# BrByte/brb_framework

Hardware: AMD Instinct MI355X
Metric: GiB/s (device-resident) + Mrecords/s over 1500B buffers at 1/2/4/8 MI355X (higher is better)
Workload: dtype u32

## Files before the change

brb_framework_amd/csrc/gpu/digest_var_line.h:

```cpp
#pragma once

#include "byte_stream.h"
#include "digest_line.h"
#include "test_options.h"

namespace brb_digest {

template <class Alg>
BRB_DEV typename Alg::State digest_lane(const uint8_t *a, uint64_t len)
{
    typename Alg::State st = Alg::iv();
    brb_io::BlockSrc src;
    src.init(a, len);
    uint32_t w[16];
    for (uint64_t b = 0; b < (len >> 6); ++b) {
        src.fetch(w);
        Alg::compress(st, w);
    }
    src.fetch(w);
    brb_io::add_marker(w, len);
    Alg::finish(st, w, uint32_t(len & 63), len);
    return st;
}

BRB_DEV uint64_t uniform64(uint64_t v)
{
    return (uint64_t(uint32_t(__builtin_amdgcn_readfirstlane(int(uint32_t(v >> 32))))) << 32) |
           uint32_t(__builtin_amdgcn_readfirstlane(int(uint32_t(v))));
}

BRB_DEV uint64_t wave_min64(uint64_t v)
{
#pragma unroll
    for (int m = 32; m >= 1; m >>= 1) {
        const uint64_t o = __shfl_xor(v, m, 64);
        v = o < v ? o : v;
    }
    return v;
}

BRB_DEV uint64_t wave_max64(uint64_t v)
{
#pragma unroll
    for (int m = 32; m >= 1; m >>= 1) {
        const uint64_t o = __shfl_xor(v, m, 64);
        v = o > v ? o : v;
    }
    return v;
}

constexpr uint32_t kSortCG = 4;
constexpr uint32_t kSortNB = 8;

BRB_DEV uint64_t sorted_record(uint64_t g, uint32_t lane, const uint32_t *__restrict__ lens, uint64_t n_rec,
                               uint32_t *scratch)
{
    const uint64_t cg = (g / kSortCG) * kSortCG;
    const uint64_t c0 = cg * 64;
    const uint64_t left = (n_rec + 63) / 64 - cg;
    const uint32_t pc = left < kSortCG ? uint32_t(left) : kSortCG;
    const uint32_t j = uint32_t((g % kSortCG + g / gridDim.x) % pc);
    uint32_t it[kSortCG];
    bool ok[kSortCG];
    uint32_t lo = 0xFFFFFFFFu, hi = 0;
#pragma unroll
    for (uint32_t v = 0; v < kSortCG; v++) {
        const uint64_t idx = c0 + 64 * v + lane;
        ok[v] = idx < n_rec;
        const uint32_t len = ok[v] ? lens[idx] : 0u;
        const uint32_t nb = (len >> 6) + ((len & 63) ? 1u : 0u);
        it[v] = (nb >> 1) + (nb & 1);
        lo = ok[v] && it[v] < lo ? it[v] : lo;
        hi = ok[v] && it[v] > hi ? it[v] : hi;
    }
#pragma unroll
    for (int m = 32; m >= 1; m >>= 1) {
        const uint32_t a = uint32_t(__shfl_xor(int(lo), m, 64)), b = uint32_t(__shfl_xor(int(hi), m, 64));
        lo = a < lo ? a : lo;
        hi = b > hi ? b : hi;
    }
    lo = __builtin_amdgcn_readfirstlane(lo);
    hi = __builtin_amdgcn_readfirstlane(hi);
    const uint32_t span = hi > lo ? hi - lo : 0u;
    const float scale = span < kSortNB ? 1.0f : float(kSortNB - 1) / float(span);
    uint32_t key[kSortCG], pos[kSortCG];
#pragma unroll
    for (uint32_t v = 0; v < kSortCG; v++) {
        const uint32_t d = it[v] - lo;
        const uint32_t q = uint32_t(float(d) * scale + 0.5f);
        key[v] = !ok[v] ? kSortNB - 1 : (q < kSortNB ? q : kSortNB - 1);
        pos[v] = 0;
    }
    uint32_t base = 0;
#pragma unroll
    for (uint32_t k = 0; k < kSortNB; k++) {
#pragma unroll
        for (uint32_t v = 0; v < kSortCG; v++) {
            const uint64_t m = __builtin_amdgcn_ballot_w64(key[v] == k);
            const uint32_t below = __builtin_amdgcn_mbcnt_hi(uint32_t(m >> 32), __builtin_amdgcn_mbcnt_lo(uint32_t(m), 0u));
            pos[v] = key[v] == k ? base + below : pos[v];
            base += uint32_t(__builtin_popcountll(m));
        }
    }
#pragma unroll
    for (uint32_t v = 0; v < kSortCG; v++)
        scratch[pos[v]] = ok[v] ? 64 * v + lane : 0xFFFFFFFFu;
    __builtin_amdgcn_s_waitcnt(0xC07F);
    __builtin_amdgcn_wave_barrier();
    const uint32_t e = scratch[64 * j + lane];
    __builtin_amdgcn_s_waitcnt(0xC07F);
    __builtin_amdgcn_wave_barrier();
    return e == 0xFFFFFFFFu ? ~uint64_t(0) : c0 + e;
}

template <class Alg, int WAVES, bool OUT_ALIGNED, bool FIXED = false, bool SORT = false>
__global__ __launch_bounds__(64 * WAVES, 2) void digest_var_line_kernel(const uint8_t *__restrict__ data,
                                                                        const uint64_t *__restrict__ offs,
                                                                        const uint32_t *__restrict__ lens,
                                                                        uint32_t rec_len, uint64_t n_rec,
                                                                        uint8_t *__restrict__ out,
                                                                        uint64_t brb_first_sorted = 0)
{
    constexpr uint32_t SLOT = 8192;
    constexpr uint32_t OOB = 0x80000000u;
    __shared__ __attribute__((aligned(16))) uint8_t ring[WAVES * 2 * SLOT];
    __shared__ uint32_t sort_scratch[SORT ? WAVES * 64 * kSortCG : 1];
    __shared__ uint32_t next_ticket;
    const uint32_t lane = threadIdx.x & 63;
    const uint32_t wv = __builtin_amdgcn_readfirstlane(threadIdx.x >> 6);
    const uint64_t n_groups = (n_rec + 63) / 64;
    if (threadIdx.x == 0)
        next_ticket = WAVES;
    __syncthreads();
    auto take = [&]() -> uint64_t {
        uint32_t tk = 0;
        if (lane == 0)
            tk = __hip_atomic_fetch_add(&next_ticket, 1u, __ATOMIC_RELAXED, __HIP_MEMORY_SCOPE_WORKGROUP);
        tk = __builtin_amdgcn_readfirstlane(tk);
        return uint64_t(blockIdx.x) + uint64_t(tk) * gridDim.x;
    };
    uint64_t g = uint64_t(blockIdx.x) + uint64_t(wv) * gridDim.x;
    if (g >= n_groups)
        return;
    const uint32_t my_off = wv * 2 * SLOT;
    const uint32_t lds0 = uint32_t(reinterpret_cast<uintptr_t>(ring)) + my_off;
    const uint64_t dbase = reinterpret_cast<uint64_t>(data);
    auto swz = [](uint32_t row) { return (row >> 1) & 7; };

    struct Grp {
        uint64_t a;
        uint64_t r;
        uint32_t len;
        uint32_t K;
        bool line;
        brb_dma::v4i rs;
        uint32_t vq[8];
        uint32_t lq[8];
    };
    const uint64_t first_sorted = brb_first_sorted;
    auto record_of = [&](uint64_t g) -> uint64_t {
        if (SORT && g >= first_sorted && g < n_groups)
            return sorted_record(g, lane, lens, n_rec, sort_scratch + wv * (64 * kSortCG));
        return g * 64 + lane < n_rec ? g * 64 + lane : ~uint64_t(0);
    };
    auto setup = [&](uint64_t g, uint64_t rec, Grp &G) {
        const uint64_t r = rec != ~uint64_t(0) ? rec : uniform64(g * 64);
        G.r = rec;
        G.a = dbase + (FIXED ? r * rec_len : offs[r]);
        G.len = FIXED ? rec_len : (rec != ~uint64_t(0) ? lens[r] : 0u);
        const uint64_t line = G.a & ~uint64_t(127);
        const uint32_t lines = G.len ? uint32_t(((G.a & 127) + G.len + 127) >> 7) : 0u;
        const uint32_t nblk = (G.len >> 6) + ((G.len & 63) ? 1u : 0u);
        const uint64_t lo = uniform64(wave_min64(G.len ? line : ~uint64_t(0)));
        const uint64_t hi = uniform64(wave_max64(G.len ? line + 128 * uint64_t(lines) : 0));
        G.K = __builtin_amdgcn_readfirstlane(uint32_t(wave_max64((nblk + 1) >> 1)));
        G.line = hi > lo && hi - lo < (uint64_t(1) << 31) - (uint64_t(1) << 16);
        const uint64_t base = lo - 4096;
        const uint64_t left = hi - base;
        G.rs.x = __builtin_amdgcn_readfirstlane(int(uint32_t(base)));
        G.rs.y = __builtin_amdgcn_readfirstlane(int(uint32_t(base >> 32) & 0xFFFF));
        G.rs.z = __builtin_amdgcn_readfirstlane(int(left > 0x7FFFFFFFull ? 0x7FFFFFFFu : uint32_t(left)));
        G.rs.w = 0x00020000;
        const uint32_t rel = uint32_t(line - lo);
        const uint32_t l3 = lane >> 3;
        const uint32_t g0 = 16u * ((lane & 7) ^ (l3 >> 1));
#pragma unroll
        for (int q = 0; q < 8; q++) {
            const int src = int(8 * q + l3) * 4;
            const uint32_t rrel = uint32_t(__builtin_amdgcn_ds_bpermute(src, int(rel)));
            G.lq[q] = uint32_t(__builtin_amdgcn_ds_bpermute(src, int(lines)));
            G.vq[q] = (rrel | (q & 1 ? g0 ^ 64u : g0)) + (4096u - 1024u * (q & 3));
        }
    };
    auto issue = [&](Grp &G, uint32_t m, uint32_t slot, bool keep_l2 = false) {
        const uint32_t lm = lds0 + slot * SLOT;
        uint32_t v[8];
#pragma unroll
        for (int q = 0; q < 8; q++)
            v[q] = m < G.lq[q] ? G.vq[q] : OOB;
        uint32_t keep;
#define BRB_VLINE_DMA8(POL)                                                                     \
        asm volatile("s_mov_b32 %0, m0\n\t"                                                    \
                     "s_mov_b32 m0, %10\n\t"                                                   \
                     "s_nop 0\n\t"                                                             \
                     "buffer_load_dwordx4 %1, %9, 0 offen " POL "lds\n\t"                      \
                     "buffer_load_dwordx4 %2, %9, 0 offen offset:1024 " POL "lds\n\t"          \
                     "buffer_load_dwordx4 %3, %9, 0 offen offset:2048 " POL "lds\n\t"          \
                     "buffer_load_dwordx4 %4, %9, 0 offen offset:3072 " POL "lds\n\t"          \
                     "s_mov_b32 m0, %11\n\t"                                                   \
                     "s_nop 0\n\t"                                                             \
                     "buffer_load_dwordx4 %5, %9, 0 offen " POL "lds\n\t"                      \
                     "buffer_load_dwordx4 %6, %9, 0 offen offset:1024 " POL "lds\n\t"          \
                     "buffer_load_dwordx4 %7, %9, 0 offen offset:2048 " POL "lds\n\t"          \
                     "buffer_load_dwordx4 %8, %9, 0 offen offset:3072 " POL "lds\n\t"          \
                     "s_mov_b32 m0, %0"                                                         \
                     : "=&s"(keep)                                                              \
                     : "v"(v[0]), "v"(v[1]), "v"(v[2]), "v"(v[3]), "v"(v[4]), "v"(v[5]), "v"(v[6]), "v"(v[7]), \
                       "s"(G.rs), "s"(lm), "s"(lm + 4096u)                                      \
                     : "memory")
        if (keep_l2)
            BRB_VLINE_DMA8("");
        else
            BRB_VLINE_DMA8("nt ");
#undef BRB_VLINE_DMA8
        const uint64_t b = ((uint64_t(uint32_t(G.rs.y)) << 32) | uint32_t(G.rs.x)) + 128u;
        G.rs.x = int(uint32_t(b));
        G.rs.y = int(uint32_t(b >> 32));
        int z = G.rs.z;
        asm("s_sub_i32 %0, %0, 0x80\n\ts_max_i32 %0, %0, 0" : "+s"(z) : : "scc");
        G.rs.z = z;
    };
    auto start = [&](Grp &G) {
        if (G.line) {
            issue(G, 0, 0, FIXED);
            issue(G, 1, 1, FIXED);
        }
    };

    uint32_t ae[33], ao[33];
    auto win_setup = [&](const Grp &G) {
        const uint32_t sh4 = uint32_t(G.a) & 124u;
        const uint32_t fr = (my_off + lane * 128) | (swz(lane) << 4);
#pragma unroll
        for (uint32_t i = 0; i < 33; i++) {
            const uint32_t q4 = sh4 + 4 * i;
            ae[i] = ((q4 & 124u) ^ fr) | ((q4 & 128u) << 6);
            ao[i] = ae[i] ^ SLOT;
            asm volatile("" : "+v"(ao[i]));
        }
    };
    uint32_t w0[16], w1[16];
    auto read_window = [&](const uint32_t (&ad)[33], uint32_t fb) {
        uint32_t d[33];
#pragma unroll
        for (int i = 0; i < 33; i++)
            d[i] = *reinterpret_cast<const uint32_t *>(ring + ad[i]);
        __builtin_amdgcn_s_waitcnt(0xC07F);
#pragma unroll
        for (int i = 0; i < 16; i++) {
            w0[i] = __builtin_amdgcn_alignbit(d[i + 1], d[i], fb);
            w1[i] = __builtin_amdgcn_alignbit(d[i + 17], d[i + 16], fb);
        }
    };

    Grp G, Gn;
    setup(g, record_of(g), G);
    start(G);
    __builtin_amdgcn_sched_barrier(0);
    for (;;) {
        const uint64_t gn = take();
        const uint64_t rn = record_of(gn);
        const uint64_t r = G.r;
        typename Alg::State st;
        if (!G.line) {
            st = digest_lane<Alg>(reinterpret_cast<const uint8_t *>(G.a), G.len);
            if (gn < n_groups) {
                setup(gn, rn, Gn);
                start(Gn);
            }
        } else {
            win_setup(G);
            const uint32_t fb = (uint32_t(G.a) & 3u) * 8u;
            const uint32_t nfull = G.len >> 6, t = G.len & 63;
            const uint32_t tb = t ? nfull : 0xFFFFFFFFu;
            uint32_t wt[16];
#pragma unroll
            for (int i = 0; i < 16; i++)
                wt[i] = 0;
            st = Alg::iv();
            const uint32_t K = G.K;
            auto step = [&](uint32_t k, const uint32_t (&ad)[33], uint32_t refill_slot) {
                brb_dma::wait_vmcnt<0>();
                read_window(ad, fb);
                if (k < K) {
                    issue(G, k + 1, refill_slot);
                } else if (gn < n_groups) {
                    setup(gn, rn, Gn);
                    start(Gn);
                }
                const uint32_t b = 2 * k - 2;
                if (b < nfull)
                    Alg::compress(st, w0);
                if (b + 1 < nfull)
                    Alg::compress(st, w1);
                if (__builtin_amdgcn_ballot_w64(tb - b < 2) != 0) {
#pragma unroll
                    for (int i = 0; i < 16; i++)
                        wt[i] = tb == b ? w0[i] : tb == b + 1 ? w1[i] : wt[i];
                }
            };
            if (K == 0) {
                brb_dma::wait_vmcnt<0>();
                if (gn < n_groups) {
                    setup(gn, rn, Gn);
                    start(Gn);
                }
            }
            for (uint32_t k = 1; k <= K; k += 2) {
                step(k, ae, 0);
                if (k == K)
                    break;
                step(k + 1, ao, 1);
            }
            if (t == 0) {
                Alg::pad_only(st, G.len);
            } else {
#pragma unroll
                for (uint32_t i = 0; i < 16; i++) {
                    const uint32_t o = 4 * i;
                    const uint32_t keep = t > o ? (t - o < 4 ? t - o : 4) : 0;
                    uint32_t v = keep == 4 ? wt[i] : wt[i] & ((1u << (8 * keep)) - 1u);
                    if (t >= o && t < o + 4)
                        v |= 0x80u << (8 * (t - o));
                    wt[i] = v;
                }
                Alg::finish(st, wt, t, G.len);
            }
        }
        if (r != ~uint64_t(0))
            Alg::template store<OUT_ALIGNED>(out, r, st);
        g = gn;
        if (g >= n_groups)
            break;
        G = Gn;
    }
}

template <class Alg>
hipError_t launch_var_line(const uint8_t *data, const uint64_t *offs, const uint32_t *lens, uint64_t n_rec, uint8_t *out,
                           bool out_al, hipStream_t s)
{
    constexpr int W = 8;
    const uint64_t groups = (n_rec + 63) / 64;
    const unsigned g = unsigned(groups < device_cu_count() ? groups : device_cu_count());
    const bool sort = brb_opt::get(brb_opt::kVarSort) != 0 && groups > uint64_t(g) * W && g % kSortCG == 0;
    const uint64_t first = brb_opt::get(brb_opt::kVarSort) == 2 ? uint64_t(g) * W : 0;
    if (sort && out_al)
        digest_var_line_kernel<Alg, W, true, false, true><<<g, 64 * W, 0, s>>>(data, offs, lens, 0, n_rec, out, first);
    else if (sort)
        digest_var_line_kernel<Alg, W, false, false, true><<<g, 64 * W, 0, s>>>(data, offs, lens, 0, n_rec, out, first);
    else if (out_al)
        digest_var_line_kernel<Alg, W, true><<<g, 64 * W, 0, s>>>(data, offs, lens, 0, n_rec, out);
    else
        digest_var_line_kernel<Alg, W, false><<<g, 64 * W, 0, s>>>(data, offs, lens, 0, n_rec, out);
    return hipGetLastError();
}

template <class Alg>
hipError_t launch_fixed_var_line(const uint8_t *data, uint32_t rec_len, uint64_t n_rec, uint8_t *out, bool out_al,
                                 hipStream_t s)
{
    constexpr int W = 8;
    const uint64_t groups = (n_rec + 63) / 64;
    const unsigned g = unsigned(groups < device_cu_count() ? groups : device_cu_count());
    if (out_al)
        digest_var_line_kernel<Alg, W, true, true><<<g, 64 * W, 0, s>>>(data, nullptr, nullptr, rec_len, n_rec, out);
    else
        digest_var_line_kernel<Alg, W, false, true><<<g, 64 * W, 0, s>>>(data, nullptr, nullptr, rec_len, n_rec, out);
    return hipGetLastError();
}

inline bool var_line_enabled()
{
    return brb_opt::get(brb_opt::kVarLine) != 0;
}

}
```

brb_framework_amd/csrc/gpu/md5_kernels.hip:

```cpp
#include "brb_kernels.h"
#include "byte_stream.h"
#include "digest_dma.h"
#include "digest_var_line.h"
#include "md5_device.h"

namespace {

struct Md5Alg;

struct Out16 {
    template <bool ALIGNED>
    static BRB_DEV void store(uint8_t *out, uint64_t r, const Md5State &st)
    {
        const uint4 v = make_uint4(st.a, st.b, st.c, st.d);
        if (ALIGNED)
            reinterpret_cast<uint4 *>(out)[r] = v;
        else
            __builtin_memcpy(out + 16 * r, &v, 16);
    }
};

struct Md5Alg {
    using State = Md5State;
    static BRB_DEV State iv() { return md5_iv(); }
    static BRB_DEV void compress(State &st, uint32_t (&w)[16]) { md5_compress(st, w); }
    static BRB_DEV void finish(State &st, uint32_t (&w)[16], uint32_t t, uint64_t len) { md5_finish(st, w, t, len); }
    static BRB_DEV void pad_only(State &st, uint64_t len) { md5_pad_only(st, len); }
    template <bool ALIGNED>
    static BRB_DEV void store(uint8_t *out, uint64_t r, const State &st) { Out16::store<ALIGNED>(out, r, st); }
};

template <int BLOCK, bool OUT_ALIGNED>
__global__ __launch_bounds__(BLOCK) void md5_fixed_a4_kernel(const uint8_t *__restrict__ data, uint32_t rec_len,
                                                              uint64_t n_rec, uint8_t *__restrict__ out)
{
    const uint64_t r = uint64_t(blockIdx.x) * BLOCK + threadIdx.x;
    if (r >= n_rec)
        return;
    const uint8_t *p = data + r * rec_len;
    const uint32_t nfull = rec_len >> 6;
    Md5State st = md5_iv();
    uint32_t w[16];

    if (nfull) {
        uint4 n0 = ld16_a4(p), n1 = ld16_a4(p + 16), n2 = ld16_a4(p + 32), n3 = ld16_a4(p + 48);
        for (uint32_t b = 0; b < nfull; ++b) {
            const uint4 c0 = n0, c1 = n1, c2 = n2, c3 = n3;
            const uint8_t *q = p + 64u * (b + 1 < nfull ? b + 1 : b);
            n0 = ld16_a4(q);
            n1 = ld16_a4(q + 16);
            n2 = ld16_a4(q + 32);
            n3 = ld16_a4(q + 48);
            w[0] = c0.x; w[1] = c0.y; w[2] = c0.z; w[3] = c0.w;
            w[4] = c1.x; w[5] = c1.y; w[6] = c1.z; w[7] = c1.w;
            w[8] = c2.x; w[9] = c2.y; w[10] = c2.z; w[11] = c2.w;
            w[12] = c3.x; w[13] = c3.y; w[14] = c3.z; w[15] = c3.w;
            md5_compress(st, w);
        }
    }
    const uint32_t t = rec_len & 63;
    const uint8_t *pt = p + 64u * nfull;
#pragma unroll
    for (uint32_t i = 0; i < 16; i++)
        w[i] = tail_word_a4(pt, t, i);
    md5_finish(st, w, t, rec_len);
    Out16::store<OUT_ALIGNED>(out, r, st);
}

template <int BLOCK, bool FIXED, bool OUT_ALIGNED>
__global__ __launch_bounds__(BLOCK) void md5_any_kernel(const uint8_t *__restrict__ data, const uint64_t *__restrict__ offs,
                                                         const uint32_t *__restrict__ lens, uint32_t rec_len,
                                                         uint64_t n_rec, uint8_t *__restrict__ out)
{
    const uint64_t r = uint64_t(blockIdx.x) * BLOCK + threadIdx.x;
    if (r >= n_rec)
        return;
    const uint8_t *a = data + (FIXED ? r * rec_len : offs[r]);
    const uint64_t len = FIXED ? rec_len : lens[r];
    const uint64_t nfull = len >> 6;
    Md5State st = md5_iv();
    uint32_t w[16];
    brb_io::BlockSrc src;
    src.init(a, len);
    for (uint64_t b = 0; b < nfull; ++b) {
        src.fetch(w);
        md5_compress(st, w);
    }
    src.fetch(w);
    brb_io::add_marker(w, len);
    md5_finish(st, w, uint32_t(len & 63), len);
    Out16::store<OUT_ALIGNED>(out, r, st);
}

constexpr int kBlock = 256;

inline unsigned grid_for(uint64_t n)
{
    return unsigned((n + kBlock - 1) / kBlock);
}

}

namespace brb {

hipError_t launch_md5_fixed(const uint8_t *data, uint32_t rec_len, uint64_t n_rec, uint8_t *out, hipStream_t s)
{
    if (n_rec == 0)
        return hipSuccess;
    const bool out_al = (reinterpret_cast<uintptr_t>(out) & 15) == 0;
    const unsigned g = grid_for(n_rec);
    const brb_digest::FixedRoute route = brb_digest::fixed_route(reinterpret_cast<uintptr_t>(data), rec_len);
    switch (route) {
    case brb_digest::kRouteLaneA4:
        if (out_al)
            md5_fixed_a4_kernel<kBlock, true><<<g, kBlock, 0, s>>>(data, rec_len, n_rec, out);
        else
            md5_fixed_a4_kernel<kBlock, false><<<g, kBlock, 0, s>>>(data, rec_len, n_rec, out);
        return hipGetLastError();
    case brb_digest::kRouteLaneAny:
        if (out_al)
            md5_any_kernel<kBlock, true, true><<<g, kBlock, 0, s>>>(data, nullptr, nullptr, rec_len, n_rec, out);
        else
            md5_any_kernel<kBlock, true, false><<<g, kBlock, 0, s>>>(data, nullptr, nullptr, rec_len, n_rec, out);
        return hipGetLastError();
    default:
        return brb_digest::launch_fixed_dma<Md5Alg>(route, data, rec_len, n_rec, out, out_al, s);
    }
}

hipError_t launch_md5_var(const uint8_t *data, const uint64_t *offs, const uint32_t *lens, uint64_t n_rec,
                          uint8_t *out, hipStream_t s)
{
    if (n_rec == 0)
        return hipSuccess;
    const bool out_al = (reinterpret_cast<uintptr_t>(out) & 15) == 0;
    if (brb_digest::var_line_enabled())
        return brb_digest::launch_var_line<Md5Alg>(data, offs, lens, n_rec, out, out_al, s);
    const unsigned g = grid_for(n_rec);
    if (out_al)
        md5_any_kernel<kBlock, false, true><<<g, kBlock, 0, s>>>(data, offs, lens, 0, n_rec, out);
    else
        md5_any_kernel<kBlock, false, false><<<g, kBlock, 0, s>>>(data, offs, lens, 0, n_rec, out);
    return hipGetLastError();
}

}
```

brb_framework_amd/csrc/gpu/sha1_device.h:

```cpp
#pragma once

#include "brb_gpu_common.h"

struct Sha1State {
    uint32_t a, b, c, d, e;
};

BRB_DEV Sha1State sha1_iv()
{
    return Sha1State{0x67452301u, 0xEFCDAB89u, 0x98BADCFEu, 0x10325476u, 0xC3D2E1F0u};
}

#define BRB_SHA1_CH(b, c, d) __builtin_amdgcn_bitop3_b32((b), (c), (d), 0xCA)
#define BRB_SHA1_PAR(b, c, d) __builtin_amdgcn_bitop3_b32((b), (c), (d), 0x96)
#define BRB_SHA1_MAJ(b, c, d) __builtin_amdgcn_bitop3_b32((b), (c), (d), 0xE8)
#define BRB_SHA1_W(i) \
    (w[(i) & 15] = rotl<1>(__builtin_amdgcn_bitop3_b32(w[((i) + 13) & 15], w[((i) + 8) & 15], w[((i) + 2) & 15], 0x96) ^ w[(i) & 15]))
#define BRB_SHA1_R(F, K, v, x, y, z, u, wi)                    \
    do {                                                       \
        (u) += F((x), (y), (z)) + (wi) + (K) + rotl<5>(v);     \
        (x) = rotl<30>(x);                                     \
    } while (0)

BRB_DEV void sha1_compress(Sha1State &st, uint32_t (&w)[16])
{
    uint32_t a = st.a, b = st.b, c = st.c, d = st.d, e = st.e;
    constexpr uint32_t K0 = 0x5A827999u, K1 = 0x6ED9EBA1u, K2 = 0x8F1BBCDCu, K3 = 0xCA62C1D6u;

#define R5(F, K, i, W)                                   \
    BRB_SHA1_R(F, K, a, b, c, d, e, W(i + 0));           \
    BRB_SHA1_R(F, K, e, a, b, c, d, W(i + 1));           \
    BRB_SHA1_R(F, K, d, e, a, b, c, W(i + 2));           \
    BRB_SHA1_R(F, K, c, d, e, a, b, W(i + 3));           \
    BRB_SHA1_R(F, K, b, c, d, e, a, W(i + 4));
#define W0(i) w[(i)]
#define WX(i) BRB_SHA1_W(i)
    R5(BRB_SHA1_CH, K0, 0, W0) R5(BRB_SHA1_CH, K0, 5, W0) R5(BRB_SHA1_CH, K0, 10, W0)
    BRB_SHA1_R(BRB_SHA1_CH, K0, a, b, c, d, e, w[15]);
    BRB_SHA1_R(BRB_SHA1_CH, K0, e, a, b, c, d, WX(16));
    BRB_SHA1_R(BRB_SHA1_CH, K0, d, e, a, b, c, WX(17));
    BRB_SHA1_R(BRB_SHA1_CH, K0, c, d, e, a, b, WX(18));
    BRB_SHA1_R(BRB_SHA1_CH, K0, b, c, d, e, a, WX(19));
    R5(BRB_SHA1_PAR, K1, 20, WX) R5(BRB_SHA1_PAR, K1, 25, WX) R5(BRB_SHA1_PAR, K1, 30, WX) R5(BRB_SHA1_PAR, K1, 35, WX)
    R5(BRB_SHA1_MAJ, K2, 40, WX) R5(BRB_SHA1_MAJ, K2, 45, WX) R5(BRB_SHA1_MAJ, K2, 50, WX) R5(BRB_SHA1_MAJ, K2, 55, WX)
    R5(BRB_SHA1_PAR, K3, 60, WX) R5(BRB_SHA1_PAR, K3, 65, WX) R5(BRB_SHA1_PAR, K3, 70, WX) R5(BRB_SHA1_PAR, K3, 75, WX)
#undef W0
#undef WX
#undef R5

    st.a += a;
    st.b += b;
    st.c += c;
    st.d += d;
    st.e += e;
}

BRB_DEV void sha1_finish(Sha1State &st, uint32_t (&w)[16], uint32_t t, uint64_t len)
{
#pragma unroll
    for (int i = 0; i < 16; i++)
        w[i] = __builtin_bswap32(w[i]);
    if (t >= 56) {
        sha1_compress(st, w);
#pragma unroll
        for (int i = 0; i < 14; i++)
            w[i] = 0;
    }
    w[14] = uint32_t(len >> 29) + (len >= (uint64_t(1) << 29) ? 1u : 0u);
    w[15] = uint32_t(len << 3);
    sha1_compress(st, w);
}

BRB_DEV void sha1_pad_only(Sha1State &st, uint64_t len)
{
    uint32_t w[16] = {0x80000000u};
    w[14] = uint32_t(len >> 29) + (len >= (uint64_t(1) << 29) ? 1u : 0u);
    w[15] = uint32_t(len << 3);
    sha1_compress(st, w);
}
```

brb_framework_amd/csrc/gpu/sha1_kernels.hip:

```cpp
#include "brb_kernels.h"
#include "byte_stream.h"
#include "digest_dma.h"
#include "digest_var_line.h"
#include "sha1_device.h"

namespace {

template <bool ALIGNED>
BRB_DEV void store20(uint8_t *out, uint64_t r, const Sha1State &st)
{
    const uint32_t v[5] = {__builtin_bswap32(st.a), __builtin_bswap32(st.b), __builtin_bswap32(st.c),
                           __builtin_bswap32(st.d), __builtin_bswap32(st.e)};
    uint8_t *o = out + 20 * r;
    if (ALIGNED) {
        uint32_t *o32 = reinterpret_cast<uint32_t *>(o);
#pragma unroll
        for (int i = 0; i < 5; i++)
            o32[i] = v[i];
    } else {
        __builtin_memcpy(o, v, 20);
    }
}

struct Sha1Alg {
    using State = Sha1State;
    static BRB_DEV State iv() { return sha1_iv(); }
    static BRB_DEV void compress(State &st, uint32_t (&w)[16])
    {
#pragma unroll
        for (int i = 0; i < 16; i++)
            w[i] = __builtin_bswap32(w[i]);
        sha1_compress(st, w);
    }
    static BRB_DEV void finish(State &st, uint32_t (&w)[16], uint32_t t, uint64_t len) { sha1_finish(st, w, t, len); }
    static BRB_DEV void pad_only(State &st, uint64_t len) { sha1_pad_only(st, len); }
    template <bool ALIGNED>
    static BRB_DEV void store(uint8_t *out, uint64_t r, const State &st) { store20<ALIGNED>(out, r, st); }
};

template <int BLOCK, bool OUT_ALIGNED>
__global__ __launch_bounds__(BLOCK) void sha1_fixed_a4_kernel(const uint8_t *__restrict__ data, uint32_t rec_len,
                                                               uint64_t n_rec, uint8_t *__restrict__ out)
{
    const uint64_t r = uint64_t(blockIdx.x) * BLOCK + threadIdx.x;
    if (r >= n_rec)
        return;
    const uint8_t *p = data + r * rec_len;
    const uint32_t nfull = rec_len >> 6;
    Sha1State st = sha1_iv();
    uint32_t w[16];

    if (nfull) {
        uint4 n0 = ld16_a4(p), n1 = ld16_a4(p + 16), n2 = ld16_a4(p + 32), n3 = ld16_a4(p + 48);
        for (uint32_t b = 0; b < nfull; ++b) {
            const uint4 c0 = n0, c1 = n1, c2 = n2, c3 = n3;
            const uint8_t *q = p + 64u * (b + 1 < nfull ? b + 1 : b);
            n0 = ld16_a4(q);
            n1 = ld16_a4(q + 16);
            n2 = ld16_a4(q + 32);
            n3 = ld16_a4(q + 48);
            w[0] = c0.x; w[1] = c0.y; w[2] = c0.z; w[3] = c0.w;
            w[4] = c1.x; w[5] = c1.y; w[6] = c1.z; w[7] = c1.w;
            w[8] = c2.x; w[9] = c2.y; w[10] = c2.z; w[11] = c2.w;
            w[12] = c3.x; w[13] = c3.y; w[14] = c3.z; w[15] = c3.w;
#pragma unroll
            for (int i = 0; i < 16; i++)
                w[i] = __builtin_bswap32(w[i]);
            sha1_compress(st, w);
        }
    }
    const uint32_t t = rec_len & 63;
    const uint8_t *pt = p + 64u * nfull;
#pragma unroll
    for (uint32_t i = 0; i < 16; i++)
        w[i] = tail_word_a4(pt, t, i);
    sha1_finish(st, w, t, rec_len);
    store20<OUT_ALIGNED>(out, r, st);
}

template <int BLOCK, bool FIXED, bool OUT_ALIGNED>
__global__ __launch_bounds__(BLOCK) void sha1_any_kernel(const uint8_t *__restrict__ data, const uint64_t *__restrict__ offs,
                                                          const uint32_t *__restrict__ lens, uint32_t rec_len,
                                                          uint64_t n_rec, uint8_t *__restrict__ out)
{
    const uint64_t r = uint64_t(blockIdx.x) * BLOCK + threadIdx.x;
    if (r >= n_rec)
        return;
    const uint8_t *a = data + (FIXED ? r * rec_len : offs[r]);
    const uint64_t len = FIXED ? rec_len : lens[r];
    const uint64_t nfull = len >> 6;
    Sha1State st = sha1_iv();
    uint32_t w[16];
    brb_io::BlockSrc src;
    src.init(a, len);
    for (uint64_t b = 0; b < nfull; ++b) {
        src.fetch(w);
#pragma unroll
        for (uint32_t i = 0; i < 16; i++)
            w[i] = __builtin_bswap32(w[i]);
        sha1_compress(st, w);
    }
    src.fetch(w);
    brb_io::add_marker(w, len);
    sha1_finish(st, w, uint32_t(len & 63), len);
    store20<OUT_ALIGNED>(out, r, st);
}

constexpr int kBlock = 256;

inline unsigned grid_for(uint64_t n)
{
    return unsigned((n + kBlock - 1) / kBlock);
}

}

namespace brb {

hipError_t launch_sha1_fixed(const uint8_t *data, uint32_t rec_len, uint64_t n_rec, uint8_t *out, hipStream_t s)
{
    if (n_rec == 0)
        return hipSuccess;
    const bool out_al = (reinterpret_cast<uintptr_t>(out) & 3) == 0;
    const unsigned g = grid_for(n_rec);
    const brb_digest::FixedRoute route = brb_digest::fixed_route(reinterpret_cast<uintptr_t>(data), rec_len);
    switch (route) {
    case brb_digest::kRouteLaneA4:
        if (out_al)
            sha1_fixed_a4_kernel<kBlock, true><<<g, kBlock, 0, s>>>(data, rec_len, n_rec, out);
        else
            sha1_fixed_a4_kernel<kBlock, false><<<g, kBlock, 0, s>>>(data, rec_len, n_rec, out);
        return hipGetLastError();
    case brb_digest::kRouteLaneAny:
        if (out_al)
            sha1_any_kernel<kBlock, true, true><<<g, kBlock, 0, s>>>(data, nullptr, nullptr, rec_len, n_rec, out);
        else
            sha1_any_kernel<kBlock, true, false><<<g, kBlock, 0, s>>>(data, nullptr, nullptr, rec_len, n_rec, out);
        return hipGetLastError();
    default:
        return brb_digest::launch_fixed_dma<Sha1Alg>(route, data, rec_len, n_rec, out, out_al, s);
    }
}

hipError_t launch_sha1_var(const uint8_t *data, const uint64_t *offs, const uint32_t *lens, uint64_t n_rec,
                           uint8_t *out, hipStream_t s)
{
    if (n_rec == 0)
        return hipSuccess;
    const bool out_al = (reinterpret_cast<uintptr_t>(out) & 3) == 0;
    if (brb_digest::var_line_enabled())
        return brb_digest::launch_var_line<Sha1Alg>(data, offs, lens, n_rec, out, out_al, s);
    const unsigned g = grid_for(n_rec);
    if (out_al)
        sha1_any_kernel<kBlock, false, true><<<g, kBlock, 0, s>>>(data, offs, lens, 0, n_rec, out);
    else
        sha1_any_kernel<kBlock, false, false><<<g, kBlock, 0, s>>>(data, offs, lens, 0, n_rec, out);
    return hipGetLastError();
}

}
```

Measured before the change: 4298.

## Streamline var-line setup with DPP reductions and fold SHA1 byteswap into window perm

Replaces 64-bit shuffle-based wave min/max with 32-bit DPP reductions relative to a reference lane. For fixed-length records it computes the line span and per-row offsets analytically, with no per-lane loads. It adds a fast issue path that skips OOB masking when every lane still has lines left, and it restricts tail capture to the last steps. For SHA1 it uses v_perm with a byte-swapping selector, so the window words come out big-endian without a separate bswap. This adds template complexity and changes the tail masking, which risks correctness bugs in edge cases.

```diff
diff --git a/brb_framework_amd/csrc/gpu/digest_var_line.h b/brb_framework_amd/csrc/gpu/digest_var_line.h
--- a/brb_framework_amd/csrc/gpu/digest_var_line.h
+++ b/brb_framework_amd/csrc/gpu/digest_var_line.h
@@ -47,6 +47,36 @@
         v = o > v ? o : v;
     }
     return v;
+}
+
+struct RedMinI32 {
+    static constexpr int id = 0x7FFFFFFF;
+    static BRB_DEV int op(int a, int b) { return a < b ? a : b; }
+};
+struct RedMaxI32 {
+    static constexpr int id = int(0x80000000u);
+    static BRB_DEV int op(int a, int b) { return a > b ? a : b; }
+};
+struct RedMinU32 {
+    static constexpr int id = -1;
+    static BRB_DEV int op(int a, int b) { return int(uint32_t(a) < uint32_t(b) ? uint32_t(a) : uint32_t(b)); }
+};
+struct RedMaxU32 {
+    static constexpr int id = 0;
+    static BRB_DEV int op(int a, int b) { return int(uint32_t(a) > uint32_t(b) ? uint32_t(a) : uint32_t(b)); }
+};
+
+template <class Red>
+BRB_DEV uint32_t wave_reduce32(uint32_t x)
+{
+    int v = int(x);
+    v = Red::op(v, __builtin_amdgcn_update_dpp(Red::id, v, 0x111, 0xF, 0xF, false));
+    v = Red::op(v, __builtin_amdgcn_update_dpp(Red::id, v, 0x112, 0xF, 0xF, false));
+    v = Red::op(v, __builtin_amdgcn_update_dpp(Red::id, v, 0x114, 0xF, 0xF, false));
+    v = Red::op(v, __builtin_amdgcn_update_dpp(Red::id, v, 0x118, 0xF, 0xF, false));
+    v = Red::op(v, __builtin_amdgcn_update_dpp(Red::id, v, 0x142, 0xA, 0xF, false));
+    v = Red::op(v, __builtin_amdgcn_update_dpp(Red::id, v, 0x143, 0xC, 0xF, false));
+    return uint32_t(__builtin_amdgcn_readlane(v, 63));
 }
 
 constexpr uint32_t kSortCG = 4;
@@ -156,6 +186,12 @@
         brb_dma::v4i rs;
         uint32_t vq[8];
         uint32_t lq[8];
+        uint32_t Lmin;
+    };
+    const uint32_t l3 = lane >> 3;
+    const uint32_t gsw = 16u * ((lane & 7) ^ (l3 >> 1));
+    auto row_voffset = [&](int q, uint32_t rrel) {
+        return (rrel | (q & 1 ? gsw ^ 64u : gsw)) + (4096u - 1024u * (q & 3));
     };
     const uint64_t first_sorted = brb_first_sorted;
     auto record_of = [&](uint64_t g) -> uint64_t {
@@ -164,42 +200,75 @@
         return g * 64 + lane < n_rec ? g * 64 + lane : ~uint64_t(0);
     };
     auto setup = [&](uint64_t g, uint64_t rec, Grp &G) {
-        const uint64_t r = rec != ~uint64_t(0) ? rec : uniform64(g * 64);
+        constexpr uint64_t kWide = (uint64_t(1) << 31) - (uint64_t(1) << 16);
         G.r = rec;
-        G.a = dbase + (FIXED ? r * rec_len : offs[r]);
-        G.len = FIXED ? rec_len : (rec != ~uint64_t(0) ? lens[r] : 0u);
-        const uint64_t line = G.a & ~uint64_t(127);
-        const uint32_t lines = G.len ? uint32_t(((G.a & 127) + G.len + 127) >> 7) : 0u;
-        const uint32_t nblk = (G.len >> 6) + ((G.len & 63) ? 1u : 0u);
-        const uint64_t lo = uniform64(wave_min64(G.len ? line : ~uint64_t(0)));
-        const uint64_t hi = uniform64(wave_max64(G.len ? line + 128 * uint64_t(lines) : 0));
-        G.K = __builtin_amdgcn_readfirstlane(uint32_t(wave_max64((nblk + 1) >> 1)));
-        G.line = hi > lo && hi - lo < (uint64_t(1) << 31) - (uint64_t(1) << 16);
-        const uint64_t base = lo - 4096;
-        const uint64_t left = hi - base;
-        G.rs.x = __builtin_amdgcn_readfirstlane(int(uint32_t(base)));
-        G.rs.y = __builtin_amdgcn_readfirstlane(int(uint32_t(base >> 32) & 0xFFFF));
-        G.rs.z = __builtin_amdgcn_readfirstlane(int(left > 0x7FFFFFFFull ? 0x7FFFFFFFu : uint32_t(left)));
         G.rs.w = 0x00020000;
-        const uint32_t rel = uint32_t(line - lo);
-        const uint32_t l3 = lane >> 3;
-        const uint32_t g0 = 16u * ((lane & 7) ^ (l3 >> 1));
-#pragma unroll
-        for (int q = 0; q < 8; q++) {
-            const int src = int(8 * q + l3) * 4;
-            const uint32_t rrel = uint32_t(__builtin_amdgcn_ds_bpermute(src, int(rel)));
-            G.lq[q] = uint32_t(__builtin_amdgcn_ds_bpermute(src, int(lines)));
-            G.vq[q] = (rrel | (q & 1 ? g0 ^ 64u : g0)) + (4096u - 1024u * (q & 3));
+        if constexpr (FIXED) {
+            const uint64_t g0 = dbase + g * 64 * rec_len;
+            const uint64_t lo = g0 & ~uint64_t(127);
+            const uint32_t og = uint32_t(g0) & 127u;
+            const uint64_t end_line = (dbase + n_rec * rec_len + 127) & ~uint64_t(127);
+            const uint64_t gend = (g0 + uint64_t(64) * rec_len + 127) & ~uint64_t(127);
+            const uint64_t hi = gend < end_line ? gend : end_line;
+            G.a = lo + (og + lane * rec_len);
+            G.len = rec_len;
+            const uint32_t nblk = (rec_len >> 6) + ((rec_len & 63) ? 1u : 0u);
+            G.K = (nblk + 1) >> 1;
+            G.Lmin = G.K;
+            G.line = true;
+            const uint64_t base = lo - 4096;
+            const uint64_t left = hi - base;
+            G.rs.x = __builtin_amdgcn_readfirstlane(int(uint32_t(base)));
+            G.rs.y = __builtin_amdgcn_readfirstlane(int(uint32_t(base >> 32) & 0xFFFF));
+            G.rs.z = __builtin_amdgcn_readfirstlane(int(uint32_t(left)));
+            const uint32_t xb = og + l3 * rec_len;
+#pragma unroll
+            for (int q = 0; q < 8; q++) {
+                const uint32_t x = xb + 8u * q * rec_len;
+                G.lq[q] = ((x & 127u) + rec_len + 127u) >> 7;
+                G.vq[q] = row_voffset(q, x & ~127u);
+            }
+        } else {
+            const bool have = rec != ~uint64_t(0);
+            const uint64_t r = have ? rec : uniform64(g * 64);
+            G.a = dbase + offs[r];
+            G.len = have ? lens[r] : 0u;
+            const uint64_t line = G.a & ~uint64_t(127);
+            const uint32_t lines = G.len ? uint32_t(((G.a & 127) + G.len + 127) >> 7) : 0u;
+            const uint32_t nblk = (G.len >> 6) + ((G.len & 63) ? 1u : 0u);
+            const uint64_t some = __builtin_amdgcn_ballot_w64(G.len != 0);
+            const uint32_t first = some ? uint32_t(__builtin_ctzll(some)) : 0u;
+            const uint64_t ref = (uint64_t(uint32_t(__builtin_amdgcn_readlane(int(uint32_t(line >> 32)), int(first)))) << 32) |
+                                 uint32_t(__builtin_amdgcn_readlane(int(uint32_t(line)), int(first)));
+            const int64_t d64 = int64_t(line - ref);
+            const int64_t e64 = d64 + int64_t(uint64_t(lines) << 7);
+            const bool far = G.len != 0 && (d64 <= -int64_t(kWide) || e64 > int64_t(kWide));
+            const bool wide = __builtin_amdgcn_ballot_w64(far) != 0;
+            const int32_t mn = int32_t(wave_reduce32<RedMinI32>(G.len ? uint32_t(d64) : uint32_t(RedMinI32::id)));
+            const int32_t mx = int32_t(wave_reduce32<RedMaxI32>(G.len ? uint32_t(e64) : uint32_t(RedMaxI32::id)));
+            G.K = wave_reduce32<RedMaxU32>((nblk + 1) >> 1);
+            G.Lmin = wave_reduce32<RedMinU32>(lines);
+            const uint32_t span = uint32_t(mx) - uint32_t(mn);
+            G.line = some != 0 && !wide && span < uint32_t(kWide);
+            const uint64_t lo = ref + uint64_t(int64_t(mn));
+            const uint64_t base = lo - 4096;
+            G.rs.x = __builtin_amdgcn_readfirstlane(int(uint32_t(base)));
+            G.rs.y = __builtin_amdgcn_readfirstlane(int(uint32_t(base >> 32) & 0xFFFF));
+            G.rs.z = __builtin_amdgcn_readfirstlane(int(G.line ? span + 4096u : 0u));
+            const uint32_t rel = uint32_t(d64) - uint32_t(mn);
+#pragma unroll
+            for (int q = 0; q < 8; q++) {
+                const int src = int(8 * q + l3) * 4;
+                const uint32_t rrel = uint32_t(__builtin_amdgcn_ds_bpermute(src, int(rel)));
+                G.lq[q] = uint32_t(__builtin_amdgcn_ds_bpermute(src, int(lines)));
+                G.vq[q] = row_voffset(q, rrel);
+            }
         }
     };
     auto issue = [&](Grp &G, uint32_t m, uint32_t slot, bool keep_l2 = false) {
         const uint32_t lm = lds0 + slot * SLOT;
-        uint32_t v[8];
-#pragma unroll
-        for (int q = 0; q < 8; q++)
-            v[q] = m < G.lq[q] ? G.vq[q] : OOB;
         uint32_t keep;
-#define BRB_VLINE_DMA8(POL)                                                                     \
+#define BRB_VLINE_DMA8(POL, v)                                                                     \
         asm volatile("s_mov_b32 %0, m0\n\t"                                                    \
                      "s_mov_b32 m0, %10\n\t"                                                   \
                      "s_nop 0\n\t"                                                             \
@@ -218,10 +287,21 @@
                      : "v"(v[0]), "v"(v[1]), "v"(v[2]), "v"(v[3]), "v"(v[4]), "v"(v[5]), "v"(v[6]), "v"(v[7]), \
                        "s"(G.rs), "s"(lm), "s"(lm + 4096u)                                      \
                      : "memory")
-        if (keep_l2)
-            BRB_VLINE_DMA8("");
-        else
-            BRB_VLINE_DMA8("nt ");
+        if (m < G.Lmin) {
+            if (keep_l2)
+                BRB_VLINE_DMA8("", G.vq);
+            else
+                BRB_VLINE_DMA8("nt ", G.vq);
+        } else {
+            uint32_t v[8];
+#pragma unroll
+            for (int q = 0; q < 8; q++)
+                v[q] = m < G.lq[q] ? G.vq[q] : OOB;
+            if (keep_l2)
+                BRB_VLINE_DMA8("", v);
+            else
+                BRB_VLINE_DMA8("nt ", v);
+        }
 #undef BRB_VLINE_DMA8
         const uint64_t b = ((uint64_t(uint32_t(G.rs.y)) << 32) | uint32_t(G.rs.x)) + 128u;
         G.rs.x = int(uint32_t(b));
@@ -258,8 +338,13 @@
         __builtin_amdgcn_s_waitcnt(0xC07F);
 #pragma unroll
         for (int i = 0; i < 16; i++) {
-            w0[i] = __builtin_amdgcn_alignbit(d[i + 1], d[i], fb);
-            w1[i] = __builtin_amdgcn_alignbit(d[i + 17], d[i + 16], fb);
+            if constexpr (Alg::kBeWindow) {
+                w0[i] = __builtin_amdgcn_perm(d[i + 1], d[i], fb);
+                w1[i] = __builtin_amdgcn_perm(d[i + 17], d[i + 16], fb);
+            } else {
+                w0[i] = __builtin_amdgcn_alignbit(d[i + 1], d[i], fb);
+                w1[i] = __builtin_amdgcn_alignbit(d[i + 17], d[i + 16], fb);
+            }
         }
     };
 
@@ -280,7 +365,9 @@
             }
         } else {
             win_setup(G);
-            const uint32_t fb = (uint32_t(G.a) & 3u) * 8u;
+            uint32_t fb = (uint32_t(G.a) & 3u) * 8u;
+            if constexpr (Alg::kBeWindow)
+                fb = Alg::window_selector(uint32_t(G.a) & 3u);
             const uint32_t nfull = G.len >> 6, t = G.len & 63;
             const uint32_t tb = t ? nfull : 0xFFFFFFFFu;
             uint32_t wt[16];
@@ -289,6 +376,7 @@
                 wt[i] = 0;
             st = Alg::iv();
             const uint32_t K = G.K;
+            const uint32_t kt = G.Lmin;
             auto step = [&](uint32_t k, const uint32_t (&ad)[33], uint32_t refill_slot) {
                 brb_dma::wait_vmcnt<0>();
                 read_window(ad, fb);
@@ -300,13 +388,13 @@
                 }
                 const uint32_t b = 2 * k - 2;
                 if (b < nfull)
-                    Alg::compress(st, w0);
+                    Alg::compress_win(st, w0);
                 if (b + 1 < nfull)
-                    Alg::compress(st, w1);
-                if (__builtin_amdgcn_ballot_w64(tb - b < 2) != 0) {
+                    Alg::compress_win(st, w1);
+                if (!FIXED && k + 1 >= kt && tb - b < 2) {
 #pragma unroll
                     for (int i = 0; i < 16; i++)
-                        wt[i] = tb == b ? w0[i] : tb == b + 1 ? w1[i] : wt[i];
+                        wt[i] = tb == b ? w0[i] : w1[i];
                 }
             };
             if (K == 0) {
@@ -325,16 +413,29 @@
             if (t == 0) {
                 Alg::pad_only(st, G.len);
             } else {
+                if constexpr (FIXED) {
+                    if (nfull & 1) {
+#pragma unroll
+                        for (int i = 0; i < 16; i++)
+                            wt[i] = w1[i];
+                    } else {
+#pragma unroll
+                        for (int i = 0; i < 16; i++)
+                            wt[i] = w0[i];
+                    }
+                }
 #pragma unroll
                 for (uint32_t i = 0; i < 16; i++) {
                     const uint32_t o = 4 * i;
                     const uint32_t keep = t > o ? (t - o < 4 ? t - o : 4) : 0;
-                    uint32_t v = keep == 4 ? wt[i] : wt[i] & ((1u << (8 * keep)) - 1u);
+                    const uint32_t low = (1u << (8 * (keep & 3))) - 1u;
+                    const uint32_t mask = keep == 4 ? 0xFFFFFFFFu : Alg::kBeWindow ? __builtin_bswap32(low) : low;
+                    uint32_t v = wt[i] & mask;
                     if (t >= o && t < o + 4)
-                        v |= 0x80u << (8 * (t - o));
+                        v |= Alg::kBeWindow ? 0x80000000u >> (8 * (t - o)) : 0x80u << (8 * (t - o));
                     wt[i] = v;
                 }
-                Alg::finish(st, wt, t, G.len);
+                Alg::finish_win(st, wt, t, G.len);
             }
         }
         if (r != ~uint64_t(0))
diff --git a/brb_framework_amd/csrc/gpu/md5_kernels.hip b/brb_framework_amd/csrc/gpu/md5_kernels.hip
--- a/brb_framework_amd/csrc/gpu/md5_kernels.hip
+++ b/brb_framework_amd/csrc/gpu/md5_kernels.hip
@@ -25,6 +25,9 @@
     static BRB_DEV State iv() { return md5_iv(); }
     static BRB_DEV void compress(State &st, uint32_t (&w)[16]) { md5_compress(st, w); }
     static BRB_DEV void finish(State &st, uint32_t (&w)[16], uint32_t t, uint64_t len) { md5_finish(st, w, t, len); }
+    static constexpr bool kBeWindow = false;
+    static BRB_DEV void compress_win(State &st, uint32_t (&w)[16]) { md5_compress(st, w); }
+    static BRB_DEV void finish_win(State &st, uint32_t (&w)[16], uint32_t t, uint64_t len) { md5_finish(st, w, t, len); }
     static BRB_DEV void pad_only(State &st, uint64_t len) { md5_pad_only(st, len); }
     template <bool ALIGNED>
     static BRB_DEV void store(uint8_t *out, uint64_t r, const State &st) { Out16::store<ALIGNED>(out, r, st); }
diff --git a/brb_framework_amd/csrc/gpu/sha1_device.h b/brb_framework_amd/csrc/gpu/sha1_device.h
--- a/brb_framework_amd/csrc/gpu/sha1_device.h
+++ b/brb_framework_amd/csrc/gpu/sha1_device.h
@@ -55,11 +55,8 @@
     st.e += e;
 }
 
-BRB_DEV void sha1_finish(Sha1State &st, uint32_t (&w)[16], uint32_t t, uint64_t len)
+BRB_DEV void sha1_finish_be(Sha1State &st, uint32_t (&w)[16], uint32_t t, uint64_t len)
 {
-#pragma unroll
-    for (int i = 0; i < 16; i++)
-        w[i] = __builtin_bswap32(w[i]);
     if (t >= 56) {
         sha1_compress(st, w);
 #pragma unroll
@@ -71,6 +68,19 @@
     sha1_compress(st, w);
 }
 
+BRB_DEV void sha1_finish(Sha1State &st, uint32_t (&w)[16], uint32_t t, uint64_t len)
+{
+#pragma unroll
+    for (int i = 0; i < 16; i++)
+        w[i] = __builtin_bswap32(w[i]);
+    sha1_finish_be(st, w, t, len);
+}
+
+BRB_DEV uint32_t sha1_be_selector(uint32_t phase)
+{
+    return 0x00010203u + 0x01010101u * phase;
+}
+
 BRB_DEV void sha1_pad_only(Sha1State &st, uint64_t len)
 {
     uint32_t w[16] = {0x80000000u};
diff --git a/brb_framework_amd/csrc/gpu/sha1_kernels.hip b/brb_framework_amd/csrc/gpu/sha1_kernels.hip
--- a/brb_framework_amd/csrc/gpu/sha1_kernels.hip
+++ b/brb_framework_amd/csrc/gpu/sha1_kernels.hip
@@ -33,6 +33,10 @@
         sha1_compress(st, w);
     }
     static BRB_DEV void finish(State &st, uint32_t (&w)[16], uint32_t t, uint64_t len) { sha1_finish(st, w, t, len); }
+    static constexpr bool kBeWindow = true;
+    static BRB_DEV uint32_t window_selector(uint32_t phase) { return sha1_be_selector(phase); }
+    static BRB_DEV void compress_win(State &st, uint32_t (&w)[16]) { sha1_compress(st, w); }
+    static BRB_DEV void finish_win(State &st, uint32_t (&w)[16], uint32_t t, uint64_t len) { sha1_finish_be(st, w, t, len); }
     static BRB_DEV void pad_only(State &st, uint64_t len) { sha1_pad_only(st, len); }
     template <bool ALIGNED>
     static BRB_DEV void store(uint8_t *out, uint64_t r, const State &st) { store20<ALIGNED>(out, r, st); }
```

Result: no change. 4335 (median of 4 runs) (+0.9%).
